# gradientpm/gvpm

Measured on AMD Instinct MI355X. Metric: photon gather+shift evaluations per second (G-BRE 3D), higher is better.
Workload: dtype f32; 1 GPU; BASELINE configs[1]: S-cbox + homogeneous medium, G-BRE 3D kernel, 512x512 frame, 1000000 photons/iter, 227 SPPM iters, initialScaleVolume 1.0; technique=bre3d, scene=cbox, photons_per_iter=1000000

## Files before the change

gvpm_amd/csrc/gather_bre.hip:

```cpp
#include <hip/hip_runtime.h>

#include <cstdlib>
#include <type_traits>

#include "device_types.h"
#include "shift_device.h"
#include "tile_walk.h"
#include "vec.h"

namespace gvpm {

struct HitGeom {
  double disk, distSqr;
};

__device__ __forceinline__ HitGeom hitGeom(f3 pf, f3 of, f3 df) {
#pragma clang fp contract(off)
  const double px = pf.x, py = pf.y, pz = pf.z;
  const double ox = of.x, oy = of.y, oz = of.z;
  const double dx = df.x, dy = df.y, dz = df.z;
  const double cx = px - ox, cy = py - oy, cz = pz - oz;
  HitGeom g;
  g.disk = cx * dx + cy * dy + cz * dz;
  const double qx = ox + dx * g.disk, qy = oy + dy * g.disk, qz = oz + dz * g.disk;
// ... 115 lines not shown
  const float band = 2e-6f * r2f;
  const double mint = (double)eps, maxt = (double)base.len - (double)eps, tE = 1e-12 * (1.0 + fabs(disk));
  bool in0 = d2 < r2f - band && disk > mint + tE && disk < maxt - tE;
  bool outside = d2 > r2f + band || disk < mint - tE;
  if (!outside && disk >= maxt - tE && d2 < r2f - band) {
    const int bx = ownBoxBand(pos, base.o, base.d, r, eps, base.len - eps);
    in0 = bx == 1;
    outside = bx == 0;
  }
  bool in = in0;
  if (use3D) {
    const float q = r2f - d2;
    const double dTup = (double)(fsqrt(fmaxf(q + band, 0.f)) * 1.000001f), dTlo = (double)(fsqrt(fmaxf(q - band, 0.f)) * 0.999999f);
    const double tLo = (disk - dTup) + 2.0 * dTlo * (double)rnd - tE, tHi = (disk - dTlo) + 2.0 * dTup * (double)rnd + tE;
    in = in0 && tLo > mint && tHi < (double)base.len;
    outside = outside || (in0 && (tHi < mint || tLo > (double)base.len));
  }
  return in ? 1 : (outside ? 0 : 2);
}

struct Acc27 {
  float v[27];
};

__device__ __forceinline__ void borderRule(const GatherArgs &a, uint32_t pix, int i, float &w) {
  const int px = (int)(pix & 0xFFFFu), py = (int)(pix >> 16);
  if ((i == GVPM_RIGHT && px == a.cfg.width - 1) || (i == GVPM_TOP && py == a.cfg.height - 1)) w = 1.f;
}

struct BaseTerms {
  f3 rel;
  double tPrime;
  float pdfCam, scale, tr;
  f3 bc;
};

template <int B, typename LDS>
__device__ __forceinline__ BaseTerms baseTerms(const GatherArgs &a, const LDS &s, f3 pos, f3 wi, f3 flux,
                                               const RayReg &base, uint32_t b) {
  BaseTerms t;
  const bool use3D = a.cfg.vol_technique == GVPM_VOL_BRE3D;
  const float r = a.radius, r2 = r * r;
  const d3 wD = tod(pos) - tod(base.o), bdD = tod(base.d);
  const double disk = dot(wD, bdD);
  const f3 perp = tof(wD - bdD * disk);
  const float distSqr = dot(perp, perp);
  t.tPrime = disk;
  float kernelVol = 3.14159265358979323846f * r2;
  t.pdfCam = 1.f;
  if (use3D) {
    const float deltaT = fsqrt(fmaxf(0.f, r2 - distSqr));
    t.tPrime = (disk - (double)deltaT) + (double)(2.f * deltaT * s.rnd[b]);
    kernelVol = (4.0f / 3.0f) * 3.14159265358979323846f * r2 * r;
    t.pdfCam = frcp(fmaxf(deltaT * 2.f, 0.0001f));
  }
  t.rel = perp + base.d * (float)(disk - t.tPrime);
  const float rr = a.cfg.path_set ? 2.f : 1.f;
  t.scale = rr * frcp(kernelVol * t.pdfCam);
  f3 trT;
  float dummy;
  mediumEval(a.med, (float)t.tPrime - a.cfg.epsilon, trT, dummy);
  t.tr = trT.x;
  const f3 sigS = mk3(a.med.sigmaS[0], a.med.sigmaS[1], a.med.sigmaS[2]);
  t.bc = (sigS * flux) * (t.tr * phaseEval(a.med.g, wi, -base.d) * t.scale) * base.eye;
  return t;
}



__device__ __forceinline__ bool branchAmbiguous(const GatherArgs &a, float y2, float r2, float tPf, float shLen) {
  if (a.cfg.reserved[4]) return true;
  return (a.cfg.use_shift_null && fabsf(y2 - r2) <= 4e-6f * r2) || fabsf(tPf - shLen) <= 4e-7f * (tPf + shLen);
}
template <int B, bool HS, typename LDS>
__device__ __forceinline__ void evalPhase1(const GatherArgs &a, LDS &s, const PhotonFront &ph, const RayReg &base,
                                           uint32_t b, Acc27 &acc, uint32_t &nNull, uint32_t &nFail, uint32_t &qMask) {
  const uint32_t pix = s.pix[b];
  const float r2 = a.radius * a.radius;
  const BaseTerms bt = baseTerms<B>(a, s, ph.pos, ph.wi, ph.flux, base, b);
  const f3 bc = bt.bc;
  acc.v[0] += bc.x;
  acc.v[1] += bc.y;
  acc.v[2] += bc.z;
  qMask = 0u;

  const f3 photonIn = mk3(a.med.sigmaS[0], a.med.sigmaS[1], a.med.sigmaS[2]) * ph.flux;
  const float tPf = (float)bt.tPrime;
  const uint32_t st = GVPM_PF_SHIFT_TYPE(ph.bits);
#pragma unroll
  for (int i = 0; i < 4; ++i) {
    const ShiftRel sh = loadShiftRel(s, i, b, base.d);
    const f3 y = bt.rel - (sh.ro + sh.rd * tPf);
    const float y2 = dot(y, y);
    const bool ambBranch = sh.valid && !(HS && st == 3u) && branchAmbiguous(a, y2, r2, tPf, sh.len);
    const bool isNull = !ambBranch && sh.valid && a.cfg.use_shift_null && y2 < r2 && tPf < sh.len;
    const f3 yp = y - sh.d * dot(y, sh.d);
    const float deltaS = fsqrt(fmaxf(0.f, r2 - dot(yp, yp)));
    const float pdfShiftPos = frcp(fmaxf(2.f * deltaS, 0.0001f));
    float wNull = 0.5f;
    if (a.cfg.use_mis)
      wNull = (pdfShiftPos == 0.f || bt.pdfCam == 0.f)
                  ? 1.f
                  : frcp(1.f + sh.sMIS * pdfShiftPos * frcp(bt.pdfCam));
    const f3 nullFlux = photonIn * (bt.tr * phaseEval(a.med.g, ph.wi, -sh.d)) * sh.eye;
    const bool wantsShift = !ambBranch && sh.valid && !isNull && sh.len >= tPf && a.cfg.debug_shift != GVPM_SHIFT_NULL;
    const bool queued = wantsShift && (st == 1u || st == 2u || (HS && st == 3u));
    nNull += isNull ? 1u : 0u;
    nFail += (wantsShift && !queued) ? 1u : 0u;
    qMask |= (queued || ambBranch) ? (1u << i) : 0u;
    float w = isNull ? wNull : 1.f;
    borderRule(a, pix, i, w);
    const float keep = (queued || ambBranch) ? 0.f : 1.f;
    const float ws = isNull ? w * bt.scale : 0.f;
    acc.v[3 + 3 * i + 0] += nullFlux.x * ws;
    acc.v[3 + 3 * i + 1] += nullFlux.y * ws;
    acc.v[3 + 3 * i + 2] += nullFlux.z * ws;
    acc.v[15 + 3 * i + 0] += bc.x * (w * keep);
    acc.v[15 + 3 * i + 1] += bc.y * (w * keep);
    acc.v[15 + 3 * i + 2] += bc.z * (w * keep);
  }
}

__global__ __launch_bounds__(256) void apply_host_shifts_kernel(GatherArgs a, const gvpm_host_shift *__restrict__ results, uint32_t n) {
  const uint32_t k = blockIdx.x * blockDim.x + threadIdx.x;
  uint32_t ok = 0, bad = 0;
  if (k < n) {
    const float4 c0 = a.reqCtx[4 * (size_t)k], c1 = a.reqCtx[4 * (size_t)k + 1], c2 = a.reqCtx[4 * (size_t)k + 2],
                 c3 = a.reqCtx[4 * (size_t)k + 3];
    const float tr = c0.x, pdfCam = c0.y, pdfShiftPos = c0.z, sMIS = c0.w, scale = c1.x;
    const f3 bc = mk3(c1.y, c1.z, c1.w), shD = mk3(c2.x, c2.y, c2.z), eye = mk3(c3.x, c3.y, c3.z);
    const uint32_t pix = __float_as_uint(c2.w);
    const int i = (int)__float_as_uint(c3.w);
    float w = 1.f;
    f3 sflux = mk3(0.f);
    bool good = false;
    if (results && results[k].ok) {
      const gvpm_host_shift r = results[k];
      const float jac = r.det_ratio;
      if (jac > 0.f && isfinite(jac)) {
        good = true;
        const f3 photonWeight = mk3(r.throughput[0], r.throughput[1], r.throughput[2]);
        const f3 wi = mk3(r.wi[0], r.wi[1], r.wi[2]);
        const f3 sigS = mk3(a.med.sigmaS[0], a.med.sigmaS[1], a.med.sigmaS[2]);
        const f3 contrib = (sigS * photonWeight) * phaseEval(a.med.g, wi, -shD);
        sflux = contrib * eye * (tr * jac);
        w = 0.5f;
        const float offsetPdf = r.pdf * pdfShiftPos;
        if (offsetPdf == 0.f) {
          w = 1.f;
          sflux = mk3(0.f);
        }
        if (a.cfg.use_mis) {
          const float basePdf = pdfCam * r.base_pdf;
          if (basePdf == 0.f) {
            w = 0.f;
          } else if (a.cfg.power_heuristic) {
            const float v = sMIS * jac * (offsetPdf / basePdf);
            w = 1.f / (1.f + v * v);
          } else {
            w = 1.f / (1.f + sMIS * offsetPdf * jac / basePdf);
          }
        }
      }
    }
    borderRule(a, pix, i, w);
    const size_t p = (size_t)(pix >> 16) * a.cfg.width + (pix & 0xFFFFu);
    const float ws = w * scale * a.iterScale, wbS = w * a.iterScale;
    float *dst = a.iter + p * 27;
    if (ws != 0.f) {
      atomicAdd(&dst[3 + 3 * i + 0], sflux.x * ws);
      atomicAdd(&dst[3 + 3 * i + 1], sflux.y * ws);
      atomicAdd(&dst[3 + 3 * i + 2], sflux.z * ws);
    }
    atomicAdd(&dst[15 + 3 * i + 0], bc.x * wbS);
    atomicAdd(&dst[15 + 3 * i + 1], bc.y * wbS);
    atomicAdd(&dst[15 + 3 * i + 2], bc.z * wbS);
    ok = good ? 1u : 0u;
    bad = good ? 0u : 1u;
  }
  const uint32_t nOk = (uint32_t)__popcll(__ballot(ok != 0u)), nBad = (uint32_t)__popcll(__ballot(bad != 0u));
  if ((threadIdx.x & 63) == 0 && (nOk | nBad)) {
    unsigned long long *row = a.stats + 8 * (size_t)(blockIdx.x % GVPM_STAT_ROWS);
    atomicAdd(&row[3], (unsigned long long)nOk);
    atomicAdd(&row[4], (unsigned long long)nBad);
  }
}
void launch_apply_host_shifts(const GatherArgs &a, const gvpm_host_shift *results, uint32_t n, hipStream_t s) {
  if (n) hipLaunchKernelGGL(apply_host_shifts_kernel, dim3((n + 255) / 256), dim3(256), 0, s, a, results, n);
}

template <int B, bool FULLVIS, bool HS, typename LDS>
__device__ __forceinline__ void evalPhase2Core(const GatherArgs &a, LDS &s, uint32_t pidx, uint32_t b, int i, f3 &sf,
                                               f3 &wb, uint32_t &nDiff, uint32_t &nFail, const float4 *ldsTri) {
  const PhotonCold ph = loadCold(a, pidx);
  const RayReg base = loadRay(s, 0, b);
  const ShiftRel sr = loadShiftRel(s, i, b, base.d);
  RayReg sh;
  sh.d = sr.d;
  sh.eye = sr.eye;
  sh.len = sr.len;
  sh.valid = sr.valid;
  const bool use3D = a.cfg.vol_technique == GVPM_VOL_BRE3D;
  const float r = a.radius, r2 = r * r;
  double tPrime;
  float pdfCam = 1.f;
  f3 rel;
  {
    const d3 wD = tod(ph.pos) - tod(base.o), bdD = tod(base.d);
    const double disk = dot(wD, bdD);
    const f3 perp = tof(wD - bdD * disk);
    tPrime = disk;
    if (use3D) {
      const float deltaT = fsqrt(fmaxf(0.f, r2 - dot(perp, perp)));
      tPrime = (disk - (double)deltaT) + (double)(2.f * deltaT * s.rnd[b]);
      pdfCam = frcp(fmaxf(deltaT * 2.f, 0.0001f));
    }
    rel = perp + base.d * (float)(disk - tPrime);
  }
  const float rr = a.cfg.path_set ? 2.f : 1.f;
  const float kernelVol = use3D ? (4.0f / 3.0f) * 3.14159265358979323846f * r2 * r : 3.14159265358979323846f * r2;
  const float scale = rr * frcp(kernelVol * pdfCam);
  f3 trT;
  float dummy;
  mediumEval(a.med, (float)tPrime - a.cfg.epsilon, trT, dummy);
  const f3 sigS = mk3(a.med.sigmaS[0], a.med.sigmaS[1], a.med.sigmaS[2]);
  const f3 bc = (sigS * ph.flux) * (trT.x * phaseEval(a.med.g, ph.wi, -base.d) * scale) * base.eye;

  const f3 basePt = base.o + base.d * (float)tPrime;
  const f3 dS = sr.ro + sr.rd * (float)tPrime;
  uint32_t amb = 0u;
  if (!(HS && GVPM_PF_SHIFT_TYPE(ph.bits) == 3u)) {
    const f3 y = rel - dS;
    const float y2 = dot(y, y), tPf = (float)tPrime;
    amb = branchAmbiguous(a, y2, r2, tPf, sh.len) ? 2u : 0u;
    const uint32_t stq = GVPM_PF_SHIFT_TYPE(ph.bits);
    const bool nullNow = a.cfg.use_shift_null && y2 < r2 && tPf < sh.len;
    const bool reconnects = sh.valid && !nullNow && sh.len >= tPf && a.cfg.debug_shift != GVPM_SHIFT_NULL && (stq == 1u || stq == 2u);
    if (!amb && !reconnects) amb = 2u;
  }
  f3 offRel = rel;
  if (!use3D) {
    f3 bs, bt, ns, nt;
    coherentFrame(base.d, bs, bt);
    coherentFrame(sh.d, ns, nt);
    offRel = ns * dot(rel, bs) + nt * dot(rel, bt) + sh.d * dot(rel, base.d);
  }
  if (a.cfg.use_shift_null) {
    const f3 bo = dS + offRel;
    const float bo2 = dot(bo, bo);
    amb |= fabsf(bo2 - r2) <= (use3D ? 4e-6f : 2e-5f) * r2 ? 8u : 0u;
    const float cosD2 = bo2 < r2 ? -2.f * dot(dS, offRel) * frcp(dot(dS, dS)) : 0.f;
    offRel = offRel + dS * cosD2;
  }
  float pdfShiftPos = 1.f;
  if (use3D) {
    const f3 op = offRel - sh.d * dot(offRel, sh.d);
    const float deltaO = fsqrt(fmaxf(0.f, r2 - dot(op, op)));
    pdfShiftPos = frcp(fmaxf(2.f * deltaO, 0.0001f));
  }
  if (HS && GVPM_PF_SHIFT_TYPE(ph.bits) == 3u) {
    const f3 shiftPt = basePt + dS;
    if (recordShiftRequest(reqSink(a), a.radius, pidx, a.setPerm[s.setBase + b], i, shiftPt + offRel, basePt, shiftPt, (float)tPrime, trT.x, pdfCam,
                           pdfShiftPos, sr.sMIS, scale, bc, sh.d, sh.eye, s.pix[b])) {
      sf = wb = mk3(0.f);
    } else {
      nFail++;
      sf = mk3(0.f);
      wb = bc;
    }
    return;
  }
  bool ok = false;
  f3 sflux;
  const f3 dProjU = ((basePt + dS) - ph.parentPos) + offRel;
  uint32_t ambVis = 0u;
  float w = shiftDiffuse<FULLVIS>(a, ph, ph.bits, dProjU, sh, base, s.edge[b], trT, pdfCam, pdfShiftPos, sflux, ok, ldsTri,
                                 sr.sMIS, &ambVis);
  if (amb | ambVis) {
    deferNote(a, GVPM_EX_KIND_BRE, a.setPerm[s.setBase + b], pidx, (uint32_t)i, amb | ambVis);
    sf = wb = mk3(0.f);
    return;
  }
  if (ok) nDiff++; else nFail++;
  borderRule(a, s.pix[b], i, w);
  const float ws = w * scale;
  sf = sflux * ws;
  wb = bc * w;
}

template <int B, typename LDS> __device__ __forceinline__ void flushAcc(LDS &s, Acc27 &acc, uint32_t beam) {
#pragma unroll
  for (int k = 0; k < 27; ++k) {
    atomicAdd(&s.acc[k][beam], (double)(acc.v[k]));
    acc.v[k] = 0.f;
  }
}

__device__ __forceinline__ void waveLdsSync() {
  __builtin_amdgcn_fence(__ATOMIC_RELEASE, "wavefront");
  __builtin_amdgcn_wave_barrier();
  __builtin_amdgcn_fence(__ATOMIC_ACQUIRE, "wavefront");
}

#ifndef GVPM_TRAV_WPB
#define GVPM_TRAV_WPB 1
#endif
constexpr int TRAV_WPB = GVPM_TRAV_WPB;
#ifndef GVPM_TRAV_MINW
#define GVPM_TRAV_MINW 5
#endif
#ifndef GVPM_TRAV_OWN_MINW
#define GVPM_TRAV_OWN_MINW 4
#endif
#ifndef GVPM_EVAL_UNIT
#define GVPM_EVAL_UNIT 1280
#endif
#ifndef GVPM_EVAL_UNIT_SMALL
#define GVPM_EVAL_UNIT_SMALL 256
#endif
constexpr uint32_t EVAL_UNIT = GVPM_EVAL_UNIT, EVAL_UNIT_SMALL = GVPM_EVAL_UNIT_SMALL;
struct alignas(16) TravLds {
  float x[STAGE], y[STAGE], z[STAGE];
  uint32_t bits[STAGE];
  uint32_t stageIdx[STAGE];
  float4 cyl[3];
};
typedef float v2f __attribute__((ext_vector_type(2)));

template <int B, bool OWN_WALK>
__global__ __launch_bounds__(64 * TRAV_WPB) __attribute__((amdgpu_waves_per_eu(OWN_WALK ? GVPM_TRAV_OWN_MINW : GVPM_TRAV_MINW))) void traverse_bre_kernel(GatherArgs a, const uint4 *__restrict__ items,
                                                          const uint2 *__restrict__ itemOff,
                                                          const uint32_t *__restrict__ itemCount, uint32_t *queueHead,
                                                          uint32_t *__restrict__ pairs, uint32_t *__restrict__ pairCnt,
                                                          uint32_t persistent, uint2 *__restrict__ units, uint32_t *unitCtl,
                                                          uint32_t unitCap) {
  constexpr int LPB = 64 / B;
  __shared__ TravLds sAll[TRAV_WPB];
  const int wv = __builtin_amdgcn_readfirstlane((int)(threadIdx.x >> 6));
  TravLds &s = sAll[wv];
  const int lane = threadIdx.x & 63;
  if (itemCount[7] != 0u) return;
  const uint32_t nItems = *itemCount;
  const int b = lane % B, sub = lane / B;
  const float r = a.radius;
  const float r2f = r * r;
  const float eps = a.cfg.epsilon;
  const uint32_t coalesceAt = a.cfg.reserved[3] ? (uint32_t)a.cfg.reserved[3] : 512u;
  unsigned long long nCand = 0;
  uint32_t nOver = 0;

  bool firstItem = true;
  for (;;) {
    uint32_t it = blockIdx.x * TRAV_WPB + (uint32_t)wv;
    if (!firstItem) {
      if (!persistent || gridDim.x * TRAV_WPB >= nItems) break;
      if (lane == 0) it = gridDim.x * TRAV_WPB + atomicAdd(queueHead, 1u);
      it = __shfl(it, 0, 64);
    }
    firstItem = false;
    it = (uint32_t)__builtin_amdgcn_readfirstlane((int)it);
    if (it >= nItems) break;
    const uint4 item = items[it];
    const uint32_t setBase = item.x, nb = item.y & 0xFFu, chunk = item.y >> 8;
    if (nb == 0) continue;
    const uint2 reg = itemOff[it];
    const uint32_t cap = reg.y;
    uint32_t *const outBase = pairs + (size_t)reg.x * 64u;
    const uint32_t outOff = (uint32_t)b * cap;
    uint32_t mine = 0;
    BaseInfo bi;
    const RayReg base = loadBaseDirect<B>(a, setBase, nb, lane, bi);
    TileWalk w;
    tileSetupFrom(a, base, base.valid, w);
    const bool beamValid = w.beamValid;
    const int cA0 = __builtin_amdgcn_readfirstlane(w.cA0), K = __builtin_amdgcn_readfirstlane(w.K);
    const float mint = eps, maxt = base.len - eps;
    const int dmax = a.cfg.max_depth > 0 ? a.cfg.max_depth - (int)bi.edge : 0x7FFFFFFF;
    const int dmin = a.cfg.min_depth != 0 ? a.cfg.min_depth - (int)bi.edge : -0x7FFFFFFF;
    const uint32_t pixParity = ((bi.pix & 0xFFFFu) + (bi.pix >> 16)) & 1u;
    const uint32_t fmask = 0x40u | (a.cfg.path_set ? (1u << GVPM_HOT_PARITY_BIT) : 0u);
    const uint32_t fwant = 0x40u | (a.cfg.path_set ? (pixParity << GVPM_HOT_PARITY_BIT) : 0u);
    const bool depthWindow = a.cfg.max_depth > 0 || a.cfg.min_depth != 0;
    int dlo = max(dmin, 0), dhi = min(dmax, 255);
    if (dhi < dlo) dlo = dhi = 256;
    const uint32_t dspan = (uint32_t)(dhi - dlo);
    const float wv1 = 1.7321f * (fmaxf(base.len, 0.f) + 3.f * r);
    const float Emax = 1.25e-6f * wv1;
    const float thrD2 = beamValid ? r2f + (4.f * r * Emax + r2f * 2e-6f) : -1.f;
    const float thrLo = mint - Emax, thrHi = maxt + 2.f * r;
    const bool prefilter = !(a.cfg.reserved[0] & 128);
    bool cylOk = false;
    if (prefilter) {
      const TileCyl c = tileCylinder(base, beamValid, fminf(thrLo, 0.f) - r, thrHi + r, r, 2.f * Emax);
      cylOk = c.ok;
      waveLdsSync();
      if (lane == 0) {
        s.cyl[0] = make_float4(c.o.x, c.o.y, c.o.z, c.R2);
        s.cyl[1] = make_float4(c.d.x, c.d.y, c.d.z, c.s0);
        s.cyl[2] = make_float4(c.s1, 0.f, 0.f, 0.f);
      }
      waveLdsSync();
    }
    const bool haveCyl = prefilter && __builtin_amdgcn_readfirstlane((int)cylOk);
    unsigned long long tested = 0;
    auto putStage = [&](uint32_t k, float4 v, uint32_t gi) {
      s.x[k] = v.x;
      s.y[k] = v.y;
      s.z[k] = v.z;
      s.bits[k] = __float_as_uint(v.w);
      s.stageIdx[k] = gi;
    };

    const bool bundle = a.grid.mode == 1;
    const uint32_t part = bundle ? (item.z >> 8) & 0xFFFu : 0u, parts = bundle ? max(item.z >> 20, 1u) : 1u;
    uint32_t winNo = 0;
    const int cBeg = max((int)(bundle ? item.z & 0xFFu : item.z), cA0),
              cEnd = min((int)item.w, __builtin_amdgcn_readfirstlane(w.cA1));
    for (int cA = cBeg; cA <= cEnd; cA += K) {
      const int cAe = min(cA + K - 1, cEnd);
      CellBox bx;
      if constexpr (OWN_WALK) {
        if (!slabBox(a, w, cA, cAe, bx)) continue;
      } else {
        const uint32_t stepIdx = (uint32_t)(cA - cA0) / (uint32_t)K;
        if (stepIdx >= a.planBoxStride) {
          nOver += lane == 0 ? 1u : 0u;
          continue;
        }
        if (!unpackCellBox(a.planBoxes[(size_t)chunk * a.planBoxStride + stepIdx], bx)) continue;
      }
      const int nranges = (bx.by1 - bx.by0 + 1) * (bx.bz1 - bx.bz0 + 1);
      for (int rbase = 0; rbase < nranges; rbase += 64) {
        uint32_t start, count;
        boxRange(a, bx, rbase + lane, nranges, start, count);
        const uint32_t incl = wave_scan_incl(count, lane);
        const uint32_t excl = incl - count;
        const uint32_t total = (uint32_t)__builtin_amdgcn_readlane((int)incl, 63);
        for (uint32_t win = 0; win < total; win += STAGE) {
          if (parts > 1u && (winNo++ % parts) != part) continue;
          waveLdsSync();
          const uint32_t nst = min((uint32_t)STAGE, total - win);
          if (total >= coalesceAt) {
#pragma unroll
            for (uint32_t k = (uint32_t)lane; k < (uint32_t)STAGE; k += 64u) {
              const uint32_t e = win + k;
              uint32_t rr = 0;
#pragma unroll
              for (uint32_t step = 32; step; step >>= 1) {
                const uint32_t cand = rr + step;
                const uint32_t v = (uint32_t)__shfl((int)excl, (int)(cand & 63u), 64);
                if (v <= e) rr = cand;
              }
              const uint32_t rStart = (uint32_t)__shfl((int)start, (int)rr, 64), rExcl = (uint32_t)__shfl((int)excl, (int)rr, 64);
              if (k < nst) {
                const uint32_t gi = rStart + (e - rExcl);
                putStage(k, a.hot[gi], gi);
              }
            }
          } else
          {
            const uint32_t lo_i = max(excl, win), hi_i = min(excl + count, win + STAGE);
            uint32_t i = lo_i;
            for (; i < hi_i; ++i) {
              const uint32_t gi = start + (i - excl);
              putStage(i - win, a.hot[gi], gi);
            }
          }
          waveLdsSync();
          uint32_t nkeep = nst;
          if (haveCyl) {
            nkeep = 0;
            const float4 c0 = s.cyl[0], c1 = s.cyl[1];
            const float cS1 = s.cyl[2].x;
            const f3 axO = mk3(c0.x, c0.y, c0.z), axD = mk3(c1.x, c1.y, c1.z);
            const float cylR2 = c0.w, cylS0 = c1.w, cylS1 = cS1;
            for (uint32_t k0 = 0; k0 < nst; k0 += 64u) {
              const uint32_t k = k0 + (uint32_t)lane;
              const bool live = k < nst;
              const float px = live ? s.x[k] : 0.f, py = live ? s.y[k] : 0.f, pz = live ? s.z[k] : 0.f;
              const uint32_t pb = live ? s.bits[k] : 0u, pi = live ? s.stageIdx[k] : 0u;
              const f3 wv = mk3(px, py, pz) - axO;
              const float sq = dot(wv, axD);
              const float d2 = dot(wv, wv) - sq * sq;
              const bool keep = live && d2 < cylR2 && sq > cylS0 && sq < cylS1 && (pb & 0x40u);
              const unsigned long long m = __ballot(keep);
              waveLdsSync();
              if (keep) {
                const uint32_t dst = nkeep + (uint32_t)__popcll(m & ((1ull << lane) - 1ull));
                s.x[dst] = px; s.y[dst] = py; s.z[dst] = pz; s.bits[dst] = pb; s.stageIdx[dst] = pi;
              }
              nkeep += (uint32_t)__popcll(m);
            }
            waveLdsSync();
          }
          if (lane < 16 && nkeep + (uint32_t)lane < ((nkeep + 15u) & ~15u)) s.x[nkeep + lane] = 3.0e38f;
          waveLdsSync();
          tested += nkeep;
          constexpr uint32_t G = 4;
          static_assert(STAGE % (G * LPB) == 0 && G == 4, "a lane reads four consecutive photons with one b128 per component");
          for (uint32_t jb = 0; jb < nkeep; jb += G * LPB) {
            const uint32_t j0 = jb + (uint32_t)sub * G;
            const float4 X = *reinterpret_cast<const float4 *>(&s.x[j0]);
            const float4 Y = *reinterpret_cast<const float4 *>(&s.y[j0]);
            const float4 Z = *reinterpret_cast<const float4 *>(&s.z[j0]);
            const uint4 Bt = *reinterpret_cast<const uint4 *>(&s.bits[j0]);
            uint32_t cm = 0;
            {
              const v2f ox = {base.o.x, base.o.x}, oy = {base.o.y, base.o.y}, oz = {base.o.z, base.o.z};
              const v2f dx = {base.d.x, base.d.x}, dy = {base.d.y, base.d.y}, dz = {base.d.z, base.d.z};
              const float xs[4] = {X.x, X.y, X.z, X.w}, ys[4] = {Y.x, Y.y, Y.z, Y.w}, zs[4] = {Z.x, Z.y, Z.z, Z.w};
              const uint32_t bs[4] = {Bt.x, Bt.y, Bt.z, Bt.w};
#pragma unroll
              for (int h = 0; h < 2; ++h) {
                const v2f wx = (v2f){xs[2 * h], xs[2 * h + 1]} - ox, wy = (v2f){ys[2 * h], ys[2 * h + 1]} - oy,
                          wz = (v2f){zs[2 * h], zs[2 * h + 1]} - oz;
                const v2f disk = wx * dx + (wy * dy + wz * dz);
                const v2f vx = wx - dx * disk, vy = wy - dy * disk, vz = wz - dz * disk;
                const v2f d2 = vx * vx + (vy * vy + vz * vz);
#pragma unroll
                for (int e = 0; e < 2; ++e) {
                  const int u = 2 * h + e;
                  uint32_t ok = (uint32_t)(d2[e] < thrD2) & (uint32_t)(disk[e] > thrLo) & (uint32_t)(disk[e] < thrHi);
                  ok &= (uint32_t)((bs[u] & fmask) == fwant);
                  if (depthWindow) ok &= (uint32_t)((uint32_t)((int)GVPM_PF_DEPTH(bs[u]) - dlo) <= dspan);
                  cm |= ok << u;
                }
              }
            }
            if (__ballot(cm != 0u)) {
              const uint32_t c = (uint32_t)__popc(cm);
              uint32_t before = 0, total = c;
              if (B <= 32) {
                const uint32_t t = (uint32_t)__shfl_xor((int)total, 32, 64);
                before += (lane & 32) ? t : 0u;
                total += t;
              }
              if (B == 16) {
                const uint32_t t = (uint32_t)__shfl_xor((int)c, 16, 64);
                const uint32_t pairSum = c + t;
                const uint32_t t2 = (uint32_t)__shfl_xor((int)pairSum, 32, 64);
                before = ((lane & 16) ? t : 0u) + ((lane & 32) ? t2 : 0u);
                total = pairSum + t2;
              }
              uint32_t off = mine + before;
              while (cm) {
                const uint32_t u = (uint32_t)__ffs(cm) - 1u;
                cm &= cm - 1u;
                if (off < cap) outBase[outOff + off] = s.stageIdx[j0 + u];
                else nOver++;
                ++off;
              }
              mine += total;
            }
          }
        }
      }
    }
    if (sub == 0) pairCnt[(size_t)it * B + b] = (uint32_t)b < nb ? min(mine, cap) : 0u;
    if (units) {
      uint32_t tot = (sub == 0 && (uint32_t)b < nb) ? min(mine, cap) : 0u;
#pragma unroll
      for (int o = 32; o > 0; o >>= 1) tot += (uint32_t)__shfl_xor((int)tot, o, 64);
      tot = (uint32_t)__builtin_amdgcn_readfirstlane((int)tot);
      if (tot) {
        const uint32_t parts = (tot + EVAL_UNIT - 1u) / EVAL_UNIT;
        const uint32_t cls = (tot + parts - 1u) / parts > EVAL_UNIT_SMALL ? 0u : 1u;
        uint32_t slot = 0;
        if (lane == 0) slot = atomicAdd(&unitCtl[cls], parts);
        slot = (uint32_t)__builtin_amdgcn_readfirstlane((int)slot);
        for (uint32_t pp = (uint32_t)lane; pp < parts; pp += 64u) {
          if (slot + pp < unitCap) units[(size_t)cls * unitCap + slot + pp] = make_uint2(it, pp | (parts << 16));
          else nOver++;
        }
      }
    }
    nCand += tested * nb;
  }
  {
#pragma unroll
    for (int o = 32; o > 0; o >>= 1) nOver += (uint32_t)__shfl_xor((int)nOver, o, 64);
    if (lane == 0 && (nCand | nOver)) {
      unsigned long long *row = statRow(a);
      atomicAdd(&row[1], nCand);
      if (nOver) atomicAdd(&row[7], (unsigned long long)nOver);
    }
  }
}

#ifndef GVPM_EVAL_MINW
#define GVPM_EVAL_MINW 3
#endif
#ifndef GVPM_EVAL_ATTR
#define GVPM_EVAL_ATTR
#endif
constexpr int SEG_STEPS = 16;
constexpr int SEG_QCAP = 1024;
template <int B> struct SegCfg {
  static constexpr int WPB = B == 16 ? 4 : (B == 32 ? 2 : 1);
  using Entry = typename std::conditional<B == 16, uint16_t, uint32_t>::type;
  static constexpr int BEAM_BITS = B == 16 ? 4 : 6;
};
template <int B> struct SegLds : RayTile<B> {
  double acc[27][B];
  uint32_t boff[B + 1];
  typename SegCfg<B>::Entry q[SEG_QCAP];
  uint32_t setBase;
};


#ifdef GVPM_EVAL_TIMING
__device__ unsigned long long gvpmEvalTiming[16];
__device__ unsigned long long gvpmEvalWaveLog[16 * 16384];
extern "C" int gvpm_debug_eval_timing(unsigned long long *out, int reset) {
  if (out && hipMemcpyFromSymbol(out, HIP_SYMBOL(gvpmEvalTiming), sizeof(gvpmEvalTiming)) != hipSuccess) return -1;
  if (out && hipMemcpyFromSymbol(out + 16, HIP_SYMBOL(gvpmEvalWaveLog), sizeof(gvpmEvalWaveLog)) != hipSuccess) return -1;
  if (reset) {
    unsigned long long z[16] = {0};
    if (hipMemcpyToSymbol(HIP_SYMBOL(gvpmEvalTiming), z, sizeof(z)) != hipSuccess) return -1;
  }
  return 0;
}
__device__ __forceinline__ unsigned long long tickNow() {
  unsigned long long t;
  asm volatile("s_waitcnt vmcnt(0) lgkmcnt(0)\n\ts_memtime %0\n\ts_waitcnt lgkmcnt(0)" : "=s"(t) : : "memory");
  return t;
}
#define TICK() tickNow()
__device__ __forceinline__ unsigned long long tickLight() {
  unsigned long long t;
  asm volatile("s_memtime %0\n\ts_waitcnt lgkmcnt(0)" : "=s"(t) : : "memory");
  return t;
}
#define LTICK() tickLight()
#else
#define TICK() 0ull
#define LTICK() 0ull
#endif

template <int B, bool FULLVIS, bool PF, bool HS = false>
__global__ __launch_bounds__(64 * SegCfg<B>::WPB, GVPM_EVAL_MINW * SegCfg<B>::WPB / 4 > 0 ? GVPM_EVAL_MINW * SegCfg<B>::WPB / 4 : 1) GVPM_EVAL_ATTR
void evaluate_bre_kernel(GatherArgs a, const uint4 *__restrict__ items, const uint2 *__restrict__ itemOff,
                             const uint32_t *__restrict__ itemCount, uint32_t *queueHead,
                             const uint32_t *__restrict__ pairs, const uint32_t *__restrict__ pairCnt,
                             uint32_t persistent, const uint2 *__restrict__ units, const uint32_t *__restrict__ unitCtl,
                             uint32_t unitCap) {
  constexpr int WPB = SegCfg<B>::WPB;
  constexpr int BB = SegCfg<B>::BEAM_BITS;
  using Entry = typename SegCfg<B>::Entry;
  __shared__ SegLds<B> sAll[WPB];
  extern __shared__ float4 sceneTri[];
  const int lane = threadIdx.x & 63, wv = threadIdx.x >> 6;
  if (itemCount[7] != 0u) return;
  SegLds<B> &s = sAll[wv];
  const float4 *ldsTri = nullptr;
  if (!FULLVIS && a.ntri <= EVAL_LDS_TRIS && !(a.cfg.reserved[0] & 16)) {
    for (uint32_t i = threadIdx.x; i < 3u * a.ntri; i += 64u * WPB) sceneTri[i] = a.tri4[i];
    ldsTri = sceneTri;
  }
  __syncthreads();
  const uint32_t nItems = *itemCount;
  const uint32_t waveId = blockIdx.x * WPB + wv, nWaves = gridDim.x * WPB;
  uint32_t nEval = 0, nNull = 0, nDiff = 0, nFail = 0;
  [[maybe_unused]] unsigned long long tk[12] = {0, 0, 0, 0, 0, 0, 0, 0, 0, 0, 0, 0};
  [[maybe_unused]] const unsigned long long tStart = TICK();
  [[maybe_unused]] unsigned long long tItemMax = 0;
#ifdef GVPM_EVAL_TIMING
  const unsigned long long wStart = wall_clock64();
  unsigned long long wLastStart = 0, lastN = 0, lastUk = 0, wLastEnd = 0, tkLast[6] = {0, 0, 0, 0, 0, 0}, suLast[4] = {0, 0, 0, 0};
#endif

  bool firstItem = true;
  for (;;) {
    [[maybe_unused]] const unsigned long long tItem = TICK();
    uint32_t it = waveId;
    if (!firstItem) {
      if (!persistent) break;
      if (lane == 0) it = nWaves + atomicAdd(queueHead, 1u);
      it = __shfl(it, 0, 64);
    }
    firstItem = false;
    it = (uint32_t)__builtin_amdgcn_readfirstlane((int)it);
    uint32_t part = 0u, parts = 1u;
    if (units) {
      const uint32_t c0 = min(unitCtl[0], unitCap), c1 = min(unitCtl[1], unitCap);
      if (it >= c0 + c1) break;
      const uint2 u = it < c0 ? units[it] : units[(size_t)unitCap + (it - c0)];
      it = u.x;
      part = u.y & 0xFFFFu;
      parts = u.y >> 16;
    }
    if (it >= nItems) break;
    const uint4 item = items[it];
    const uint32_t setBase = item.x, nb = item.y & 0xFFu;
    if (nb == 0) continue;
    const uint32_t cntb = (uint32_t)lane < nb ? pairCnt[(size_t)it * B + lane] : 0u;
    const uint32_t incl = wave_scan_incl(cntb, lane);
    const uint32_t total = (uint32_t)__builtin_amdgcn_readlane((int)incl, 63);
    if (total == 0) continue;
    const uint32_t per = (total + parts - 1u) / parts;
    const uint32_t r0 = part * per;
    if (r0 >= total) continue;
    const uint32_t n = min(per, total - r0);
#ifdef GVPM_EVAL_TIMING
    wLastStart = wall_clock64();
    lastN = n;
    lastUk = it;
    for (int k = 1; k <= 5; ++k) tkLast[k] = tk[k];
    const unsigned long long su0 = TICK();
#endif
    const uint2 reg = itemOff[it];
    const uint32_t *lists = pairs + (size_t)reg.x * 64u;
    const uint32_t cap = reg.y;
    waveLdsSync();
    if (lane < B) s.boff[lane + 1] = incl;
    if (lane == 0) s.boff[0] = 0u;
    if (lane == 0) s.setBase = setBase;
#ifdef GVPM_EVAL_TIMING
    const unsigned long long su1 = TICK();
#endif
    loadTileRaysNoSync<B>(a, s, setBase, nb, lane);
#ifdef GVPM_EVAL_TIMING
    const unsigned long long su2 = TICK();
#endif
    for (int idx = lane; idx < 27 * B; idx += 64) (&s.acc[0][0])[idx] = 0.0;
    waveLdsSync();
    relToBase<B>(s, lane);
    waveLdsSync();
#ifdef GVPM_EVAL_TIMING
    suLast[0] = su0 - tItem; suLast[1] = su1 - su0; suLast[2] = su2 - su1; suLast[3] = TICK() - su2;
#endif
    [[maybe_unused]] unsigned long long tMark = TICK();
    tk[1] += tMark - tItem;
    tk[6] += 1;

    const bool use3D = a.cfg.vol_technique == GVPM_VOL_BRE3D;
    const uint32_t chunk = (n + 63u) / 64u;
    const uint32_t g0 = r0 + min(n, (uint32_t)lane * chunk), g1 = min(r0 + n, g0 + chunk);
    uint32_t cur = 0;
    if (g0 < g1)
      while (s.boff[cur + 1] <= g0) cur++;

    for (uint32_t tSeg = 0; tSeg < chunk;) {
      {
        uint32_t qn = 0;
        Acc27 acc;
#pragma unroll
        for (int k = 0; k < 27; ++k) acc.v[k] = 0.f;
        bool dirty = false;
        const uint32_t tLim = chunk;
        uint32_t t = tSeg;
        auto locate = [&](uint32_t tt, uint32_t from, bool &hv, uint32_t &gg, uint32_t &bb, uint32_t &pi) {
          gg = g0 + tt;
          hv = gg < g1 && tt < tLim;
          bb = from;
          pi = 0u;
          if (hv) {
            while (s.boff[bb + 1] <= gg) bb++;
            pi = lists[(size_t)bb * cap + (gg - s.boff[bb])];
          }
        };
        bool haveN = false, haveB = false;
        uint32_t gN = 0, bN = 0, pidxN = 0, gB = 0, bB = 0, pidxB = 0;
        locate(t, cur, haveN, gN, bN, pidxN);
        PhotonFront phN = {};
        if (PF) {
          locate(t + 1u, bN, haveB, gB, bB, pidxB);
          phN = loadFront(a, pidxN);
        }
        for (; t < tLim && t - tSeg < (uint32_t)SEG_STEPS && qn + 256u <= (uint32_t)SEG_QCAP; ++t) {
          [[maybe_unused]] const unsigned long long l0 = LTICK();
          const bool have = haveN;
          const uint32_t b = bN, pidx = pidxN;
          const PhotonFront phCur = phN;
          if (PF) {
            haveN = haveB; gN = gB; bN = bB; pidxN = pidxB;
            phN = loadFront(a, pidxN);
            locate(t + 2u, bN, haveB, gB, bB, pidxB);
          } else {
            locate(t + 1u, b, haveN, gN, bN, pidxN);
          }
          [[maybe_unused]] const unsigned long long l1 = LTICK();
          tk[7] += l1 - l0;
          uint32_t qMask = 0;
          [[maybe_unused]] unsigned long long l2 = l1, l3 = l1;
          if (have) {
            if (b != cur) {
              if (dirty) flushAcc<B>(s, acc, cur);
              dirty = false;
              cur = b;
            }
            l2 = LTICK();
            const PhotonFront ph = PF ? phCur : loadFront(a, pidx);
            const RayReg base = loadRay(s, 0, cur);
            int dec = decidePair(ph.pos, base, s.rnd[cur], a.radius, a.cfg.epsilon, use3D);
            if (dec == 2) dec = decidePairFine(ph.pos, base, s.rnd[cur], a.radius, a.cfg.epsilon, use3D);
#ifdef GVPM_EVAL_TIMING
            asm volatile("" :: "v"(dec));
            l3 = LTICK();
#endif
            if (dec == 1) {
              evalPhase1<B, HS>(a, s, ph, base, cur, acc, nNull, nFail, qMask);
              dirty = true;
              nEval++;
            } else if (dec == 2) {
              deferNote(a, GVPM_EX_KIND_BRE_PAIR, a.setPerm[s.setBase + cur], pidx, 0u, 1u);
            }
          }
          const uint32_t ent = ((t - tSeg) << (8 + BB)) | ((uint32_t)lane << (2 + BB)) | cur;
#pragma unroll
          for (uint32_t i = 0; i < 4u; ++i) {
            const bool qd = (qMask >> i) & 1u;
            const unsigned long long m = __ballot(qd);
            if (qd) s.q[qn + __popcll(m & ((1ull << lane) - 1ull))] = (Entry)(ent | (i << BB));
            qn += (uint32_t)__popcll(m);
          }
#ifdef GVPM_EVAL_TIMING
          { const unsigned long long l5 = LTICK(); tk[8] += l2 - l1; tk[9] += l3 - l2; tk[10] += l5 - l3; tk[11] += 1; }
#endif
        }
        if (dirty) flushAcc<B>(s, acc, cur);
        const uint32_t tEnd = t;
        waveLdsSync();
        { [[maybe_unused]] const unsigned long long tn = TICK(); tk[2] += tn - tMark; tMark = tn; }
        const uint32_t cq = (qn + 63u) / 64u;
        const uint32_t e0 = min(qn, (uint32_t)lane * cq), e1 = min(qn, e0 + cq);
        uint32_t key = 0xFFFFFFFFu;
        f3 rs = mk3(0.f), rw = mk3(0.f);
        auto entry = [&](uint32_t j, bool &hv, uint32_t &k2o, uint32_t &pi, uint32_t &bo, uint32_t &io) {
          hv = j < cq && e0 + j < e1;
          k2o = 0xFFFFFFFFu;
          pi = bo = io = 0u;
          if (hv) {
            const uint32_t e = s.q[e0 + j];
            bo = e & ((1u << BB) - 1u);
            io = (e >> BB) & 3u;
            const uint32_t ln = (e >> (2 + BB)) & 63u, ts = e >> (8 + BB);
            const uint32_t g = r0 + min(n, ln * chunk) + tSeg + ts;
            pi = lists[(size_t)bo * cap + (g - s.boff[bo])];
            k2o = (bo << 2) | io;
          }
        };
        bool haveE = false, haveF = false;
        uint32_t k2E = 0, pidxE = 0, bE = 0, iE = 0, k2F = 0, pidxF = 0, bF = 0, iF = 0;
        entry(0u, haveE, k2E, pidxE, bE, iE);
        if (PF) entry(1u, haveF, k2F, pidxF, bF, iF);
        for (uint32_t j = 0; j <= cq; ++j) {
          const bool have = haveE;
          const uint32_t k2 = k2E, pidx = pidxE, b = bE, i = iE;
          [[maybe_unused]] float warm = 0.f;
          if (PF) {
            haveE = haveF; k2E = k2F; pidxE = pidxF; bE = bF; iE = iF;
            warm = reinterpret_cast<const float *>(a.cold + (size_t)pidxE * GVPM_REC_QUADS)[0];
            entry(j + 2u, haveF, k2F, pidxF, bF, iF);
          } else {
            entry(j + 1u, haveE, k2E, pidxE, bE, iE);
          }
          if (k2 != key && key != 0xFFFFFFFFu) {
            const uint32_t kb = key >> 2, ki = key & 3u;
            atomicAdd(&s.acc[3 + 3 * ki + 0][kb], (double)rs.x);
            atomicAdd(&s.acc[3 + 3 * ki + 1][kb], (double)rs.y);
            atomicAdd(&s.acc[3 + 3 * ki + 2][kb], (double)rs.z);
            atomicAdd(&s.acc[15 + 3 * ki + 0][kb], (double)rw.x);
            atomicAdd(&s.acc[15 + 3 * ki + 1][kb], (double)rw.y);
            atomicAdd(&s.acc[15 + 3 * ki + 2][kb], (double)rw.z);
            rs = rw = mk3(0.f);
          }
          key = k2;
          if (have) {
            f3 sf, wb;
            evalPhase2Core<B, FULLVIS, HS>(a, s, pidx, b, (int)i, sf, wb, nDiff, nFail, ldsTri);
            rs = rs + sf;
            rw = rw + wb;
          }
// ... 288 lines not shown
```

Measured before the change: 6408 Mevals/s.

## Cut VGPR pressure in BRE traversal kernel and raise occupancy target

Raises the traversal kernel's waves-per-EU hint from 5 to 6. To fit that budget, it uses empty asm barriers to rematerialise lane-derived values and to keep radius and epsilon in scalar registers inside the loop instead of holding them live. Ray origin and direction are packed into three v2f registers rather than six broadcast pairs. The cross-lane prefix sums switch from __shfl_xor to permlane32/16 swap builtins, and a redundant shuffle after readfirstlane is removed. The risk is that the tighter register budget causes spills or that the asm barriers block useful compiler optimisations.

```diff
diff --git a/gvpm_amd/csrc/gather_bre.hip b/gvpm_amd/csrc/gather_bre.hip
--- a/gvpm_amd/csrc/gather_bre.hip
+++ b/gvpm_amd/csrc/gather_bre.hip
@@ -441,12 +441,30 @@
   __builtin_amdgcn_fence(__ATOMIC_ACQUIRE, "wavefront");
 }
 
+__device__ __forceinline__ uint32_t laneXor32(uint32_t x) {
+  const auto r = __builtin_amdgcn_permlane32_swap(x, x, false, false);
+  return r[0] + r[1] - x;
+}
+__device__ __forceinline__ uint32_t laneXor16(uint32_t x) {
+  const auto r = __builtin_amdgcn_permlane16_swap(x, x, false, false);
+  return r[0] + r[1] - x;
+}
+
+__device__ __forceinline__ int freshV(int x) {
+  asm volatile("" : "+v"(x));
+  return x;
+}
+__device__ __forceinline__ float freshS(float x) {
+  asm volatile("" : "+s"(x));
+  return x;
+}
+
 #ifndef GVPM_TRAV_WPB
 #define GVPM_TRAV_WPB 1
 #endif
 constexpr int TRAV_WPB = GVPM_TRAV_WPB;
 #ifndef GVPM_TRAV_MINW
-#define GVPM_TRAV_MINW 5
+#define GVPM_TRAV_MINW 6
 #endif
 #ifndef GVPM_TRAV_OWN_MINW
 #define GVPM_TRAV_OWN_MINW 4
@@ -481,9 +499,6 @@
   if (itemCount[7] != 0u) return;
   const uint32_t nItems = *itemCount;
   const int b = lane % B, sub = lane / B;
-  const float r = a.radius;
-  const float r2f = r * r;
-  const float eps = a.cfg.epsilon;
   const uint32_t coalesceAt = a.cfg.reserved[3] ? (uint32_t)a.cfg.reserved[3] : 512u;
   unsigned long long nCand = 0;
   uint32_t nOver = 0;
@@ -494,7 +509,6 @@
     if (!firstItem) {
       if (!persistent || gridDim.x * TRAV_WPB >= nItems) break;
       if (lane == 0) it = gridDim.x * TRAV_WPB + atomicAdd(queueHead, 1u);
-      it = __shfl(it, 0, 64);
     }
     firstItem = false;
     it = (uint32_t)__builtin_amdgcn_readfirstlane((int)it);
@@ -502,6 +516,8 @@
     const uint4 item = items[it];
     const uint32_t setBase = item.x, nb = item.y & 0xFFu, chunk = item.y >> 8;
     if (nb == 0) continue;
+    const float r = freshS(a.radius), eps = freshS(a.cfg.epsilon);
+    const float r2f = r * r;
     const uint2 reg = itemOff[it];
     const uint32_t cap = reg.y;
     uint32_t *const outBase = pairs + (size_t)reg.x * 64u;
@@ -541,6 +557,7 @@
       waveLdsSync();
     }
     const bool haveCyl = prefilter && __builtin_amdgcn_readfirstlane((int)cylOk);
+    v2f oxy = {base.o.x, base.o.y}, ozdx = {base.o.z, base.d.x}, dyz = {base.d.y, base.d.z};
     unsigned long long tested = 0;
     auto putStage = [&](uint32_t k, float4 v, uint32_t gi) {
       s.x[k] = v.x;
@@ -563,7 +580,7 @@
       } else {
         const uint32_t stepIdx = (uint32_t)(cA - cA0) / (uint32_t)K;
         if (stepIdx >= a.planBoxStride) {
-          nOver += lane == 0 ? 1u : 0u;
+          nOver += freshV(lane) == 0 ? 1u : 0u;
           continue;
         }
         if (!unpackCellBox(a.planBoxes[(size_t)chunk * a.planBoxStride + stepIdx], bx)) continue;
@@ -580,8 +597,9 @@
           waveLdsSync();
           const uint32_t nst = min((uint32_t)STAGE, total - win);
           if (total >= coalesceAt) {
-#pragma unroll
-            for (uint32_t k = (uint32_t)lane; k < (uint32_t)STAGE; k += 64u) {
+            const uint32_t lane0 = (uint32_t)freshV(lane);
+#pragma unroll
+            for (uint32_t k = lane0; k < (uint32_t)STAGE; k += 64u) {
               const uint32_t e = win + k;
               uint32_t rr = 0;
 #pragma unroll
@@ -609,12 +627,13 @@
           uint32_t nkeep = nst;
           if (haveCyl) {
             nkeep = 0;
+            const int laneP = freshV(lane);
             const float4 c0 = s.cyl[0], c1 = s.cyl[1];
             const float cS1 = s.cyl[2].x;
             const f3 axO = mk3(c0.x, c0.y, c0.z), axD = mk3(c1.x, c1.y, c1.z);
             const float cylR2 = c0.w, cylS0 = c1.w, cylS1 = cS1;
             for (uint32_t k0 = 0; k0 < nst; k0 += 64u) {
-              const uint32_t k = k0 + (uint32_t)lane;
+              const uint32_t k = k0 + (uint32_t)laneP;
               const bool live = k < nst;
               const float px = live ? s.x[k] : 0.f, py = live ? s.y[k] : 0.f, pz = live ? s.z[k] : 0.f;
               const uint32_t pb = live ? s.bits[k] : 0u, pi = live ? s.stageIdx[k] : 0u;
@@ -625,7 +644,7 @@
               const unsigned long long m = __ballot(keep);
               waveLdsSync();
               if (keep) {
-                const uint32_t dst = nkeep + (uint32_t)__popcll(m & ((1ull << lane) - 1ull));
+                const uint32_t dst = nkeep + (uint32_t)__popcll(m & ((1ull << laneP) - 1ull));
                 s.x[dst] = px; s.y[dst] = py; s.z[dst] = pz; s.bits[dst] = pb; s.stageIdx[dst] = pi;
               }
               nkeep += (uint32_t)__popcll(m);
@@ -645,8 +664,11 @@
             const uint4 Bt = *reinterpret_cast<const uint4 *>(&s.bits[j0]);
             uint32_t cm = 0;
             {
-              const v2f ox = {base.o.x, base.o.x}, oy = {base.o.y, base.o.y}, oz = {base.o.z, base.o.z};
-              const v2f dx = {base.d.x, base.d.x}, dy = {base.d.y, base.d.y}, dz = {base.d.z, base.d.z};
+              asm volatile("" : "+v"(oxy), "+v"(ozdx), "+v"(dyz));
+              const v2f ox = __builtin_shufflevector(oxy, oxy, 0, 0), oy = __builtin_shufflevector(oxy, oxy, 1, 1),
+                        oz = __builtin_shufflevector(ozdx, ozdx, 0, 0);
+              const v2f dx = __builtin_shufflevector(ozdx, ozdx, 1, 1), dy = __builtin_shufflevector(dyz, dyz, 0, 0),
+                        dz = __builtin_shufflevector(dyz, dyz, 1, 1);
               const float xs[4] = {X.x, X.y, X.z, X.w}, ys[4] = {Y.x, Y.y, Y.z, Y.w}, zs[4] = {Z.x, Z.y, Z.z, Z.w};
               const uint32_t bs[4] = {Bt.x, Bt.y, Bt.z, Bt.w};
 #pragma unroll
@@ -669,15 +691,15 @@
             if (__ballot(cm != 0u)) {
               const uint32_t c = (uint32_t)__popc(cm);
               uint32_t before = 0, total = c;
-              if (B <= 32) {
-                const uint32_t t = (uint32_t)__shfl_xor((int)total, 32, 64);
-                before += (lane & 32) ? t : 0u;
-                total += t;
+              if constexpr (B == 32) {
+                const uint32_t t = laneXor32(c);
+                before = (lane & 32) ? t : 0u;
+                total = c + t;
               }
-              if (B == 16) {
-                const uint32_t t = (uint32_t)__shfl_xor((int)c, 16, 64);
+              if constexpr (B == 16) {
+                const uint32_t t = laneXor16(c);
                 const uint32_t pairSum = c + t;
-                const uint32_t t2 = (uint32_t)__shfl_xor((int)pairSum, 32, 64);
+                const uint32_t t2 = laneXor32(pairSum);
                 before = ((lane & 16) ? t : 0u) + ((lane & 32) ? t2 : 0u);
                 total = pairSum + t2;
               }
@@ -695,7 +717,10 @@
         }
       }
     }
-    if (sub == 0) pairCnt[(size_t)it * B + b] = (uint32_t)b < nb ? min(mine, cap) : 0u;
+    {
+      const int laneT = freshV(lane), bT = laneT % B;
+      if (laneT / B == 0) pairCnt[(size_t)it * B + bT] = (uint32_t)bT < nb ? min(mine, cap) : 0u;
+    }
     if (units) {
       uint32_t tot = (sub == 0 && (uint32_t)b < nb) ? min(mine, cap) : 0u;
 #pragma unroll
@@ -707,7 +732,7 @@
         uint32_t slot = 0;
         if (lane == 0) slot = atomicAdd(&unitCtl[cls], parts);
         slot = (uint32_t)__builtin_amdgcn_readfirstlane((int)slot);
-        for (uint32_t pp = (uint32_t)lane; pp < parts; pp += 64u) {
+        for (uint32_t pp = (uint32_t)freshV(lane); pp < parts; pp += 64u) {
           if (slot + pp < unitCap) units[(size_t)cls * unitCap + slot + pp] = make_uint2(it, pp | (parts << 16));
           else nOver++;
         }
```

Result: no change. 6387 Mevals/s (-0.3%).
